# akanazawa/human_dynamics

Hardware: AMD Instinct MI355X
Metric: frames/sec/GPU (ResNet+temporal+SMPL, 224x224); SMPL verts max-abs-err (higher is better)
Workload: dtype f16x3

## Files before the change

### human_dynamics_amd/build.py

```python
from __future__ import annotations

import os
import subprocess
import sys
from concurrent.futures import ThreadPoolExecutor

HERE = os.path.dirname(os.path.abspath(__file__))
CSRC = os.path.join(HERE, "csrc")
INCLUDE = os.path.join(os.path.dirname(HERE), "include")
LIB = os.path.join(HERE, "libhmmr_hip.so")
SOURCES = ["api.cpp", "pack.cpp", "gemm_conv.hip", "conv3x3_stream.hip", "conv1x1_stream.hip", "stem.hip", "bottleneck.hip", "bottleneck_split.hip", "unit_pair.hip", "b1_unit.hip", "resnet.hip", "temporal.hip", "ief.hip", "ief_grad.hip", "movie_grad.hip", "smpl.hip", "smpl_grad.hip", "losses.hip", "eval_metrics.hip", "preprocess.hip", "tube.hip", "track.hip", "handoff.hip", "render.hip", "collage.hip", "person_view.hip", "windows.hip", "video_plan.cpp", "video.cpp", "probe.hip"]
HIPCC = os.environ.get("HIPCC", "/opt/rocm/bin/hipcc")
FLAGS = ["--offload-arch=gfx950", "-O3", "-std=c++17", "-fPIC", "-fno-slp-vectorize", "-I", INCLUDE, "-I", CSRC,
         "-Wall", "-Wno-unused-function"]


EXTRA_FLAGS = {"pack.cpp": ["-ffp-contract=off"], "track.hip": ["-ffp-contract=off"], "collage.hip": ["-ffp-contract=off"],
               "tube.hip": ["-ffp-contract=off"], "person_view.hip": ["-ffp-contract=off"]}


def _newer(src, dst):
    return (not os.path.exists(dst)) or os.path.getmtime(src) > os.path.getmtime(dst)


def _deps():
    return sorted(os.path.join(d, h) for d in (CSRC, INCLUDE) for h in os.listdir(d) if h.endswith(".h"))


def build(force=False, verbose=True):
    objs, jobs = [], []
    for src in SOURCES:
        s = os.path.join(CSRC, src)
        o = os.path.join(CSRC, os.path.splitext(src)[0] + ".o")
        objs.append(o)
# ... 34 lines not shown
```

### human_dynamics_amd/csrc/conv_tiles.h

```cpp
#pragma once
#include <stdio.h>

#include "hmmr_hip.h"


#define HMMR_GENERIC_TILES(X)                                                                                                         \
    X(1, 128, 128, 2, 2, 2, 0, 128, 0, 1, "128x128, 4 waves of 64x64")                                                                \
    X(2, 128, 64, 2, 2, 2, 0, 0, 0, 2, "128x64, 4 waves of 64x32")                                                                    \
    X(3, 64, 64, 2, 2, 2, 0, 0, 3, 3, "64x64, 4 waves of 32x32")                                                                      \
    X(5, 128, 128, 4, 2, 2, 0, 128, 1, 5, "128x128, 8 waves of 32x64, two workgroups per CU")                                         \
    X(6, 128, 64, 4, 2, 2, 0, 0, 2, 6, "128x64, 8 waves of 32x32, two workgroups per CU")                                             \
     \
     \
    X(7, 256, 128, 4, 2, 3, 0, 128, 0, 7, "256x128, 8 waves of 64x64, 3-stage ring, ping-pong wave groups")                           \
    X(8, 128, 256, 2, 4, 3, 256, 256, 0, 8, "128x256, likewise: half the A rows, half the fused-preact work per MFMA; the faster 3x3 tile")

#define HMMR_PATCH_TILES(X)                                                                                                           \
    X(9, 256, 128, 4, 2, 0, 128, 128, 1, 7, "256x128, the structure of tile 7 with the A operand out of an input patch")              \
    X(10, 128, 256, 2, 4, 0, 256, 256, 0, 8, "128x256, the structure of tile 8 likewise")                                             \
    X(11, 256, 128, 4, 2, 1, 128, 128, 0, 0, "256x128 without a load segment: two fragment sets per wave, one barrier per K step")

#define HMMR_S3_TILES(X)                                                                                                              \
    X(12, 7, 2, 2, 2, 28, 0, 128, 0, 1, 8, "448 pixels, waves 2 x 2")                                                                 \
    X(13, 4, 2, 2, 2, 28, 0, 128, 0, 2, 5, "256 pixels, waves 2 x 2")                                                                 \
    X(14, 8, 2, 2, 2, 28, 0, 128, 0, 0, 6, "512 pixels, waves 2 x 2")                                                                 \
    X(15, 6, 2, 2, 2, 28, 0, 128, 0, 3, 3, "384 pixels, waves 2 x 2")                                                                 \
    X(16, 5, 2, 2, 2, 28, 0, 128, 0, 4, 1, "320 pixels, waves 2 x 2")                                                                 \
    X(17, 4, 4, 4, 1, 28, 0, 128, 0, 0, 2, "512 pixels, the waves split the pixels")                                                  \
    X(18, 3, 4, 4, 1, 28, 0, 128, 0, 0, 7, "384 pixels, the waves split the pixels")                                                  \
    X(19, 5, 2, 4, 1, 56, 0, 64, 0, 8, 5, "640 pixels x 64 channels")                                                                 \
    X(20, 4, 2, 4, 1, 56, 0, 64, 0, 9, 6, "512 pixels x 64 channels")                                                                 \
    X(21, 7, 1, 1, 4, 28, 1, 128, 0, 5, 11, "224 pixels, every wave all of them and 32 of the 128 channels")                          \
     \
     \
    X(27, 2, 2, 2, 2, 28, 1, 128, 0, 6, 4, "128 pixels, waves 2 x 2: short launches")                                                 \
    X(28, 3, 2, 2, 2, 28, 1, 128, 0, 7, 9, "192 pixels, waves 2 x 2: short launches")

#define HMMR_S1_TILES(X)                                                                                                              \
    X(22, 7, 1, 1, 4, 6, 1, 0, 128, 0, 4, 5, "224 pixels, every wave all of them and 32 of the 128 channels")                         \
    X(23, 8, 1, 1, 4, 6, 1, 0, 128, 0, 5, 6, "256 pixels, likewise")                                                                  \
    X(24, 7, 2, 2, 2, 4, 1, 1, 128, 0, 2, 3, "448 pixels, waves 2 x 2")                                                               \
    X(25, 4, 2, 2, 2, 6, 1, 1, 128, 0, 1, 1, "256 pixels, waves 2 x 2")                                                               \
    X(26, 4, 2, 2, 2, 3, 2, 1, 128, 0, 3, 2, "256 pixels, waves 2 x 2, TWO workgroups per CU (rings 3 deep, 256 registers per wave)") \
     \
    X(29, 2, 2, 2, 2, 6, 1, 0, 128, 0, 6, 4, "128 pixels, waves 2 x 2: short launches")

#define HMMR_TILE_F_MOVIE 8

namespace conv_tiles {

constexpr hmmr_conv_tile_info_t make_row(int id, int family, int fm, int fn, int wgm, int wgn, int depth, int occ, int wmax, int split_only,
                                         int conv3_form, int cols, int tune, int rank, int cand, const char* text) {
    return {id, family, fm, fn, wgm, wgn, 32 * wgm * fm, 32 * wgn * fn, wgm * fm, depth, occ, wmax, split_only, conv3_form, cols, tune, cols == 64, rank, cand, text};
}

constexpr hmmr_conv_tile_info_t kRows[] = {
#define X(ID, BM, BN, WGM, WGN, NSTAGE, COLS, TUNE, RANK, CAND, TEXT) \
    make_row(ID, HMMR_TILE_GENERIC, BM / (32 * WGM), BN / (32 * WGN), WGM, WGN, NSTAGE, NSTAGE >= 3 ? 1 : 2, 0, 0, 0, COLS, TUNE, RANK, CAND, TEXT),
    HMMR_GENERIC_TILES(X)
#undef X
#define X(ID, BM, BN, WGM, WGN, PIPE, COLS, TUNE, RANK, CAND, TEXT) \
    make_row(ID, HMMR_TILE_PATCH, BM / (32 * WGM), BN / (32 * WGN), WGM, WGN, 3, 1, 0, PIPE, 0, COLS, TUNE, RANK, CAND, TEXT),
    HMMR_PATCH_TILES(X)
#undef X
#define X(ID, FM, FN, WGM, WGN, WMAX, SPLIT_ONLY, COLS, TUNE, RANK, CAND, TEXT) \
    make_row(ID, HMMR_TILE_STREAM_3X3, FM, FN, WGM, WGN, 0, 1, WMAX, SPLIT_ONLY, 0, COLS, TUNE, RANK, CAND, TEXT),
    HMMR_S3_TILES(X)
#undef X
#define X(ID, FM, FN, WGM, WGN, D, OCC, C3, COLS, TUNE, RANK, CAND, TEXT) \
    make_row(ID, HMMR_TILE_STREAM_1X1, FM, FN, WGM, WGN, D, OCC, 0, 0, C3, COLS, TUNE, RANK, CAND, TEXT),
    HMMR_S1_TILES(X)
#undef X
};
constexpr int kCount = (int)(sizeof(kRows) / sizeof(kRows[0]));

constexpr bool well_formed() {
    for (int i = 0; i < kCount; ++i) {
        const auto& a = kRows[i];
        if (a.tile < 1 || a.tile > HMMR_CONV_TILE_MAX || a.rank < 0 || a.candidate < 0) return false;
        int ranked_rows = 0;
        for (int j = 0; j < kCount; ++j) {
            const auto& b = kRows[j];
            if (b.family == a.family && b.rank > 0) ++ranked_rows;
            if (i == j) continue;
            if (a.tile == b.tile) return false;
            if (a.family != b.family) continue;
            if (a.rank && a.rank == b.rank) return false;
            if (a.candidate && a.candidate == b.candidate && a.narrow == b.narrow) return false;
        }
        if (a.rank > ranked_rows) return false;
    }
    return true;
}
static_assert(well_formed(), "conv_tiles.h: a tile number, a rank or a tuner candidate is used twice, or a number is out of range");

inline const hmmr_conv_tile_info_t* row(int tile) {
    for (const auto& r : kRows)
        if (r.tile == tile) return &r;
    return nullptr;
}

struct Ranked { int idx[kCount]; int n; };
constexpr Ranked ranked(int family) {
    Ranked o = {};
    for (int rank = 1; rank <= kCount; ++rank)
        for (int i = 0; i < kCount; ++i)
            if (kRows[i].family == family && kRows[i].rank == rank) o.idx[o.n++] = i;
    return o;
}

inline const char* list(int family, int narrow, char* buf, size_t n) {
    size_t at = 0;
    buf[0] = 0;
    for (int t = 1, end = 0; t <= HMMR_CONV_TILE_MAX; t = end + 1) {
        const auto in = [&](int id) { const auto* r = row(id); return r && r->family == family && (narrow < 0 || r->narrow == narrow); };
        end = t;
        if (!in(t)) continue;
        while (in(end + 1)) ++end;
        const int w = snprintf(buf + at, n - at, end >= t + 2 ? "%s%d .. %d" : end > t ? "%s%d, %d" : "%s%d", at ? ", " : "", t, end);
        if (w < 0 || (size_t)w >= n - at) break;
        at += (size_t)w;
    }
    return buf;
}
// ... 8 lines not shown
    int ksteps;
};
inline int family_of(int k_order, int filter_1x1) {
    return k_order == 2 ? (filter_1x1 ? HMMR_TILE_STREAM_1X1 : HMMR_TILE_STREAM_3X3) : k_order ? HMMR_TILE_PATCH : HMMR_TILE_GENERIC;
}
inline const char* family_name(int family) {
    static const char* const name[] = {"k_order 0", "k_order 1", "k_order 2", "k_order 2 (1x1)"};
    return name[family];
}

inline int fit(int tile, const Problem& p, char* why, size_t n) {
    const int fam = family_of(p.k_order, p.filter_1x1);
    const hmmr_conv_tile_info_t* t = row(tile);
    char ids[96];
    if (!t || t->family != fam) {
        snprintf(why, n, "%s runs tiles %s, not %d", family_name(fam), list(fam, -1, ids, sizeof ids), tile);
        return -1;
    }
    if (p.cout != 0 && (t->cols == 64 ? p.cout != 64 : t->cols && p.cout % t->cols)) {
        snprintf(why, n, "%s, tile %d (%s) needs cout %s %d, not %d (filter rows are padded to 128)", family_name(fam), tile, t->text,
                 t->cols == 64 ? "=" : "a multiple of", t->cols, p.cout);
        return -1;
    }
    if (t->split_only && p.dtype >= 0 && p.dtype != HMMR_F16X3) {
        snprintf(why, n, "%s, tile %d (%s) is built for split (f16x3) operands", family_name(fam), tile, t->text);
        return -1;
    }
    if (t->wmax && p.win > t->wmax) {
        snprintf(why, n, "%s, tile %d takes images up to %d pixels wide, not %d", family_name(fam), tile, t->wmax, p.win);
        return -1;
    }
    if (p.conv3_form && fam == HMMR_TILE_STREAM_1X1 && !t->conv3_form) {
        snprintf(why, n, "%s: tile %d (%s) has no conv3 form (res / out2 / in2)", family_name(fam), tile, t->text);
        return -1;
    }
    if (fam == HMMR_TILE_STREAM_1X1 && p.ksteps > 0 && p.ksteps < t->depth) {
        snprintf(why, n, "%s: cin must be at least %d channels for tile %d (rings %d K steps deep)", family_name(fam), 16 * t->depth, tile, t->depth);
        return -1;
    }
    return 0;
}

inline int tile_for(int k_order, int filter_1x1, int conv3_form, int cout, int dtype, int candidate) {
    const int fam = family_of(k_order, filter_1x1);
    const int narrow = fam == HMMR_TILE_STREAM_3X3 && cout == 64;
    const hmmr_conv_tile_info_t* t = nullptr;
    for (const auto& r : kRows)
        if (candidate > 0 && r.family == fam && r.narrow == narrow && r.candidate == candidate) { t = &r; break; }
    if (!t) t = row(candidate);
    if (!t || t->family != fam || t->narrow != narrow) return 0;
    if (t->split_only && dtype == HMMR_BF16) return 0;
    if (conv3_form && fam == HMMR_TILE_STREAM_1X1 && !t->conv3_form) return 0;
    if (t->tune_cols && cout % t->tune_cols) return 0;
    return t->tile;
}


inline int choose_generic(long long M, int cout, int slices) {
    constexpr Ranked rk = ranked(HMMR_TILE_GENERIC);
    for (int i = 0; i + 1 < rk.n; ++i) {
        const auto& r = kRows[rk.idx[i]];
        const long long tiles = ((M + r.pixels - 1) / r.pixels) * ((cout + r.channels - 1) / r.channels);
        const bool whole = r.channels < 128 || (cout >= r.channels && cout % r.channels == 0);
        if (whole && tiles * slices >= 192) return r.tile;
    }
    return kRows[rk.idx[rk.n - 1]].tile;
}

inline int choose_patch() { return kRows[ranked(HMMR_TILE_PATCH).idx[0]].tile; }

inline int choose_s3(long long M, int cout, bool split) {
    constexpr Ranked rk = ranked(HMMR_TILE_STREAM_3X3);
    const int narrow = cout == 64;
    const long long rbs = (M + 31) / 32, nts = narrow ? 1 : cout / 128;
    int tile = 0;
    double best = 0;
    for (int i = 0; i < rk.n; ++i) {
        const auto& r = kRows[rk.idx[i]];
        if (r.narrow != narrow || (r.split_only && !split)) continue;
        const long long tiles = ((rbs + r.row_blocks - 1) / r.row_blocks) * nts;
        const double cost = (double)((tiles + 255) / 256) * (r.row_blocks + 1.5);
        if (!tile || cost < best) { tile = r.tile; best = cost; }
    }
    return tile;
}

inline int choose_s1(long long M, int cout, int nk, bool c3) {
    constexpr Ranked rk = ranked(HMMR_TILE_STREAM_1X1);
    const long long rbs = (M + 31) / 32, tiles_n = cout / 128;
    int tile = 0;
    double best = 0;
    for (int i = 0; i < rk.n; ++i) {
        const auto& r = kRows[rk.idx[i]];
        if (nk < r.depth || (c3 && !r.conv3_form)) continue;
        const long long tiles = ((rbs + r.row_blocks - 1) / r.row_blocks) * tiles_n;
        double cost = (double)((tiles + 255) / 256) * (r.row_blocks + 1.5) * (r.tile == 22 || r.tile == 23 ? 1.15 : 1.0);
        if (r.tile == 26) cost = (double)((tiles + 511) / 512) * 2.0 * (r.row_blocks + 1.5) * (c3 ? 0.8 : nk <= 32 ? 0.88 : 1.05);
        if (!tile || cost < best) { tile = r.tile; best = cost; }
    }
    return tile;
}

constexpr int s1_min_depth() {
    int d = 1 << 30;
    for (const auto& r : kRows)
        if (r.family == HMMR_TILE_STREAM_1X1 && r.depth < d) d = r.depth;
    return d;
}

// ... 2 lines not shown
```

### human_dynamics_amd/csrc/gemm_conv.hip

```cpp
#include <stdlib.h>
#include <string.h>
#include <type_traits>

#include "conv_tiles.h"
#include "stream_kit.h"

struct ConvArgs {
    const void* in; const void* w; const float* scale; const float* shift;
    const void* res; void* out; void* out2; const float* scale2; const float* shift2;
    const float* pro_scale; const float* pro_shift;
    void* out_b; int ldo_b, n_split, relu_b;
    int M, K, cout, ldo, ldr;
    int Wo, HoWo, Hin, Win;
    long long in_img_stride; int in_row_stride, in_px_stride;
    int cin_log2, KH, KW, SY, SX, PY, PX;
    int res_strided; long long res_img_stride; int res_row_stride, res_px_stride;
    int relu, tiles_n, n_tiles;
    int kt_per_slice;
    long long out_slice_stride;
    int probe;
    const void* in2; int cin2, kt_split;
    int batch; long long bz_in, bz_w, bz_out, bz_res, bz_scale, bz_shift;
};

// ... 875 lines not shown
#undef X
        default: hmmr_set_error("hmmr_conv_gemm: k_order 1: no tile %d", tile); return -1;
    }
}

template <typename TA, typename TO, int BM, int BN, int WGM, int WGN, bool PRO, bool UTAP, int NSTAGE>
static int launch_cfg(const ConvArgs& base, int slices, hipStream_t stream) {
    ConvArgs a = base;
    const int tiles_m = (a.M + BM - 1) / BM;
    a.tiles_n = (a.cout + BN - 1) / BN;
    a.n_tiles = tiles_m * a.tiles_n;
    constexpr int kring = NSTAGE * (BM + BN) * 128, epi = BM * BN * 4;
    const int kloop = kring + ((PRO && NSTAGE >= 3) ? 8 * a.K : 0);
    const int lds = kloop > epi ? kloop : epi;
    if (lds > 160 * 1024) { hmmr_set_error("hmmr_conv_gemm: tile needs %d B of LDS (K = %d)", lds, a.K); return -1; }
    auto kern = conv_gemm_kernel<TA, TO, BM, BN, WGM, WGN, PRO, UTAP, NSTAGE>;
    static DeviceOnce once;
    constexpr int BKE_ = 8 * elem_traits<TA>::EPS;
    const int nk = a.K / BKE_;
    a.kt_per_slice = (nk + slices - 1) / slices;
    return launch_with_lds(kern, once, dim3(a.n_tiles, slices, a.batch), dim3(WGM * WGN * 64), NSTAGE >= 3 ? 160 * 1024 : lds, lds, stream, a);
}

template <typename TA, typename TO, bool PRO, bool UTAP>
static int launch_tiled(const ConvArgs& a, int tile, int slices, hipStream_t stream) {
    switch (tile) {
#define X(ID, BM, BN, WGM, WGN, NSTAGE, ...) case ID: return launch_cfg<TA, TO, BM, BN, WGM, WGN, PRO, UTAP, NSTAGE>(a, slices, stream);
        HMMR_GENERIC_TILES(X)
#undef X
        default: hmmr_set_error("hmmr_conv_gemm: k_order 0: no tile %d", tile); return -1;
    }
}

template <typename TA, typename TO>
static int launch_typed(const ConvArgs& a, int tile, int slices, hipStream_t stream) {
    if (tile == 0) tile = conv_tiles::choose_generic(a.M, a.cout, slices);
    char why[256];
    HMMR_REQUIRE(!conv_tiles::fit(tile, conv_tiles::Problem{0, 0, 0, a.cout, -1, 0, 0}, why, sizeof why), "hmmr_conv_gemm: %s", why);
    const bool utap = ((size_t)1 << a.cin_log2) * sizeof(TA) >= 128;
    if (a.pro_scale) {
        if (!utap) { hmmr_set_error("hmmr_conv_gemm: fused pre-activation needs cin*sizeof >= 128"); return -1; }
        return launch_tiled<TA, TO, true, true>(a, tile, slices, stream);
    }
    return utap ? launch_tiled<TA, TO, false, true>(a, tile, slices, stream)
                : launch_tiled<TA, TO, false, false>(a, tile, slices, stream);
}

template <typename TO>
__global__ __launch_bounds__(256) void splitk_reduce_kernel(const ConvArgs a0, const float* __restrict__ part,
                                                            int slices, int ldw, long long plane) {
// ... 57 lines not shown
#pragma unroll
        for (int j = 0; j < 8; ++j) {
            const float vr = stored_value<TO>(v[j]);
            u[j] = fmaxf(fmaf(vr, s2[j], b2[j]), 0.f);
        }
        if (full) store8(out2 + oo, u);
        else store_tail(out2 + oo, u, a.cout - n);
    }
}

extern "C" size_t hmmr_conv_splitk_workspace_bytes(int m, int cout, int split_k) {
    if (split_k <= 1 || m <= 0) return 0;
    return (size_t)split_k * (size_t)m * (size_t)((cout + 127) / 128 * 128) * sizeof(float);
}

static int ilog2_exact(int v) {
    int l = 0;
    while ((1 << l) < v) ++l;
    return ((1 << l) == v) ? l : -1;
}

int hmmr_conv3x3_stream(const hmmr_conv_desc_t* d, hipStream_t stream);
int hmmr_conv1x1_stream(const hmmr_conv_desc_t* d, hipStream_t stream);

extern "C" int hmmr_conv_gemm(const hmmr_conv_desc_t* d, void* stream) {
    HMMR_REQUIRE(d && d->in && d->w && (d->out || d->out2), "hmmr_conv_gemm: null operand");
    const int esz = d->in_dtype == HMMR_BF16 ? 2 : 4;
    const int eps = d->in_dtype == HMMR_F16X3 ? 8 : 16 / esz;
    const int cl2 = ilog2_exact(d->cin);
    HMMR_REQUIRE(cl2 >= 0 && d->cin % eps == 0, "hmmr_conv_gemm: cin=%d must be a power of two >= %d", d->cin, eps);
    const int K = d->kh * d->kw * d->cin + (d->in2 ? d->cin2 : 0);
    HMMR_REQUIRE(d->kh * d->kw <= 32, "hmmr_conv_gemm: at most 32 filter taps");
    const int bke = 128 / esz;
    HMMR_REQUIRE(K % bke == 0, "hmmr_conv_gemm: K=%d must be a multiple of %d", K, bke);
    HMMR_REQUIRE(d->out_dtype != HMMR_F16X3 || d->cout % 8 == 0,
                 "hmmr_conv_gemm: a split (f16x3) output needs cout %% 8 == 0 (rows are whole hi/lo groups)");
    HMMR_REQUIRE(d->ldo % 8 == 0, "hmmr_conv_gemm: ldo=%d must be a multiple of 8", d->ldo);
    const bool px_ok = d->in_px_stride % eps == 0 ||
                       (d->kw == 1 && d->px == 0 && (d->in_px_stride * d->sx) % eps == 0);
    HMMR_REQUIRE(px_ok && d->in_row_stride % eps == 0 && d->in_img_stride % eps == 0,
                 "hmmr_conv_gemm: input strides must keep 16-byte alignment");
    HMMR_REQUIRE(!d->res || d->res_strided || d->ldr % 8 == 0, "hmmr_conv_gemm: ldr must be a multiple of 8");
    HMMR_REQUIRE(!d->res || d->cout % 8 == 0 || (!d->res_strided && d->ldr >= (d->cout + 7) / 8 * 8),
                 "hmmr_conv_gemm: residual rows must be readable up to cout rounded up to 8");
    HMMR_REQUIRE(!d->out2 || (d->scale2 && d->shift2), "hmmr_conv_gemm: out2 needs scale2/shift2");
    HMMR_REQUIRE(!d->pro_scale == !d->pro_shift, "hmmr_conv_gemm: pro_scale and pro_shift go together");
// ... 18 lines not shown
    a.pro_scale = d->pro_scale; a.pro_shift = d->pro_shift;
    a.out_b = d->out_b; a.ldo_b = d->ldo_b; a.n_split = d->n_split; a.relu_b = d->relu_b;
    a.M = d->n_img * d->ho * d->wo; a.K = K; a.cout = d->cout; a.ldo = d->ldo; a.ldr = d->ldr;
    a.Wo = d->wo; a.HoWo = d->ho * d->wo; a.Hin = d->hin; a.Win = d->win;
    a.in_img_stride = d->in_img_stride; a.in_row_stride = d->in_row_stride; a.in_px_stride = d->in_px_stride;
    a.cin_log2 = cl2; a.KH = d->kh; a.KW = d->kw; a.SY = d->sy; a.SX = d->sx; a.PY = d->py; a.PX = d->px;
    a.res_strided = d->res_strided; a.res_img_stride = d->res_img_stride;
    a.res_row_stride = d->res_row_stride; a.res_px_stride = d->res_px_stride;
    a.relu = d->relu; a.tiles_n = 0; a.n_tiles = 0;
    a.kt_per_slice = 0; a.out_slice_stride = 0; a.probe = 0;
    a.in2 = d->in2; a.cin2 = d->in2 ? d->cin2 : 0; a.kt_split = d->cin / bke;
    a.batch = d->batch > 1 ? d->batch : 1;
    a.bz_in = d->batch_in_bytes; a.bz_w = d->batch_w_bytes; a.bz_out = d->batch_out_bytes;
    a.bz_res = d->batch_res_bytes; a.bz_scale = d->batch_scale_bytes; a.bz_shift = d->batch_shift_bytes;
    HMMR_REQUIRE(a.batch == 1 || (a.batch <= 64 && !d->k_order && !d->out_b && !d->in2 && !d->pro_scale &&
                                  ((d->batch_in_bytes | d->batch_w_bytes | d->batch_out_bytes | d->batch_res_bytes | d->batch_scale_bytes | d->batch_shift_bytes) & 15) == 0),
                 "hmmr_conv_gemm: a grouped launch (batch > 1) takes up to 64 problems, strides that are multiples of 16 bytes, "
                 "and no k_order / out_b / in2 / pro_scale");
#ifdef HMMR_GEMM_PROBE
    a.probe = hmmr_debug_state()->gemm_probe;
#endif
    if (a.M <= 0) return 0;
    hipStream_t s = (hipStream_t)stream;
    if (d->k_order == 2 && d->kh == 1 && d->kw == 1) return hmmr_conv1x1_stream(d, s);
    if (d->k_order) {
        HMMR_REQUIRE((d->k_order == 1 || d->k_order == 2) && d->kh == 3 && d->kw == 3 && d->sy == 1 && d->sx == 1 && d->py == 1 && d->px == 1 &&
                     d->ho == d->hin && d->wo == d->win && d->in_px_stride == d->cin && d->in_row_stride == d->win * d->cin &&
                     d->in_img_stride == (int64_t)d->hin * d->win * d->cin && (d->cin * esz) % 128 == 0 &&
                     !d->res && !d->out2 && !d->out_b && !d->pro_scale && !d->in2 && d->split_k <= 1 && d->out && d->cout % 8 == 0,
                     "hmmr_conv_gemm: k_order 1 is for 3x3 / stride 1 / pad 1 convolutions over a dense NHWC tensor with "
                     "cin a multiple of the 128-byte K step and a scale/shift/relu epilogue (no res, out2, out_b, pro_scale, in2, split_k)");
        if (d->k_order == 2) return hmmr_conv3x3_stream(d, s);
        const bool px3 = d->in_dtype == HMMR_F16X3 && d->out_dtype == HMMR_F16X3, pbf = d->in_dtype == HMMR_BF16 && d->out_dtype == HMMR_BF16;
        HMMR_REQUIRE(px3 || pbf, "hmmr_conv_gemm: k_order 1 is built for split (f16x3) and bf16 tensors");
        const int ptile = d->tile ? d->tile : conv_tiles::choose_patch();
        HMMR_REQUIRE(!conv_tiles::fit(ptile, conv_tiles::Problem{1, 0, 0, d->cout, d->in_dtype, 0, 0}, why, sizeof why), "hmmr_conv_gemm: %s", why);
        if (pbf) return launch_patch_tiled<bf16_t, bf16_t>(a, ptile, s);
        return launch_patch_tiled<bsplit_t, bsplit_t>(a, ptile, s);
    }
    const bool in16 = d->in_dtype == HMMR_BF16, in32 = d->in_dtype == HMMR_F32, inx3 = d->in_dtype == HMMR_F16X3;
    const bool out16 = d->out_dtype == HMMR_BF16, out32 = d->out_dtype == HMMR_F32, outx3 = d->out_dtype == HMMR_F16X3;
    HMMR_REQUIRE((in16 || in32 || inx3) && (out16 || out32 || outx3), "hmmr_conv_gemm: unsupported dtypes %d -> %d", d->in_dtype, d->out_dtype);
    const int nk = K / bke;
    int slices = d->split_k > 1 ? d->split_k : 1;
    if (slices > nk) slices = nk;
    slices = (nk + ((nk + slices - 1) / slices) - 1) / ((nk + slices - 1) / slices);
// ... 33 lines not shown
```

### human_dynamics_amd/csrc/resnet.hip

```cpp
#include <stdlib.h>

#include <type_traits>

#include "common.h"
#include "hmmr_hip.h"
#include "workspace.h"

int hmmr_stem_fused(const float* images, int n_real, int n, const void* wts, const float* wscale, const float* bias,
                    const float* pscale, const float* pshift, void* out, int dtype, hipStream_t s,
                    const void* w1, const float* s1, const float* b1, void* out_h1);

static constexpr int IMG = 224, PADH = 230, PADW = 232;

__global__ void stem_repack_split_kernel(const float* __restrict__ img, bsplit_t* __restrict__ out, long long npairs,
                                         long long n_real) {
    for (long long i = (long long)blockIdx.x * blockDim.x + threadIdx.x; i < npairs;
         i += (long long)gridDim.x * blockDim.x) {
        const int xp = (int)(i % (PADW / 2));
        const long long t = i / (PADW / 2);
        const int y = (int)(t % PADH);
        const long long n = t / PADH;
        float v[8];
#pragma unroll
        for (int e = 0; e < 8; ++e) v[e] = 0.f;
        const int sy = y - 3;
        if (n < n_real && (unsigned)sy < (unsigned)IMG) {
#pragma unroll
// ... 329 lines not shown
        const T* res = p.shortcut == HMMR_SC_NONE ? X[cur] : xn;
        const int res_stride = p.shortcut == HMMR_SC_NONE ? U.stride : 1;
        hmmr_conv_desc_t d;
        if (p.shortcut == HMMR_SC_LAUNCH || p.shortcut == HMMR_SC_LAUNCH_WITH_CONV1) {
            d = dense_conv(dt, n, xin, H, U.c_in, 1, U.stride, U.depth, U.shortcut, xn);
            d.pro_scale = ps; d.pro_shift = pb;
            d.k_order = 0;
            if (p.shortcut == HMMR_SC_LAUNCH_WITH_CONV1) {
                d.w = U.sc_c1.w; d.scale = U.sc_c1.scale; d.shift = U.sc_c1.shift; d.k_order = U.sc_c1.k_order;
                d.cout = U.depth + U.base; d.out_b = T1; d.ldo_b = U.base; d.n_split = U.depth; d.relu_b = 1;
            }
            if (hmmr_conv_gemm(&d, s)) return -2;
        }
        if (p.shortcut != HMMR_SC_NONE && prof_mark(pf)) return -2;
        if (p.conv1 == HMMR_CONV1_LAUNCH) {
            d = dense_conv(dt, n, xin, H, U.c_in, 1, 1, U.base, U.conv1, T1);
            d.pro_scale = ps; d.pro_shift = pb; d.relu = 1;
            if (hmmr_conv_gemm(&d, s)) return -2;
        }
        if (prof_mark(pf)) return -2;
        if (p.conv2 == HMMR_CONV2_LAUNCH) {
            d = dense_conv(dt, n, T1, H, U.base, 3, U.stride, U.base, U.conv2, T2);
            d.relu = 1;
            if (hmmr_conv_gemm(&d, s)) return -2;
        }
        if (prof_mark(pf)) return -2;
        if (p.end == HMMR_END_CONV3_LAUNCH) {
            d = dense_conv(dt, n, T2, Ho, U.base, 1, 1, U.depth, sc_in_c3 ? U.c3sc : U.conv3, out);
            if (sc_in_c3) { d.in2 = xin; d.cin2 = U.c_in; } else set_residual(d, res, U.depth, H, res_stride);
            if (pre) { d.out2 = pre; d.scale2 = N.pre_scale; d.shift2 = N.pre_shift; }
            if (hmmr_conv_gemm(&d, s)) return -2;
        } else {
            hmmr_tail_desc_t t = {};
            t.dtype = dt; t.m = n * Ho * Ho; t.c_mid = U.base; t.depth = U.depth; t.ho = t.wo = Ho;
            t.w3 = U.conv3.w; t.scale3 = U.conv3.scale; t.shift3 = U.conv3.shift;
            if (p.conv2 == HMMR_CONV2_IN_TAIL) {
                t.h1 = T1; t.hin = t.win = H; t.w2 = U.conv2.w; t.scale2 = U.conv2.scale; t.shift2 = U.conv2.shift;
            } else t.h2 = T2;
            if (p.end == HMMR_END_TAIL_BF16_STRIDE2) {
                t.conv2_stride = U.stride;
                set_residual(t, res, U.depth, H, res_stride);
                t.out = out; t.out_pre = pre;
                if (pre) { t.pre_scale = N.pre_scale; t.pre_shift = N.pre_shift; }
            } else {
                if (dt == HMMR_F16X3) {
                    t.w3 = U.w3_frag;
// ... 71 lines not shown
```

Before: 39310.

## Add dedicated streaming kernel for stride-2 3x3 convolutions on split tensors

Adds a new kernel for 3x3 stride-2 pad-1 convolutions on f16x3 tensors. It streams filter and input pixel slabs into LDS rings several stages deep with direct global-to-LDS loads, zero-pads the top and left edges from a zero page, and interleaves fragment reads with MFMAs. Adds tile rows and a chooser for it. Dispatch sends matching convolutions with no tile set to it by default, in place of the generic implicit GEMM path. This adds a large hand-scheduled kernel with tight vmcnt and LDS budget assumptions.

```diff
diff --git a/human_dynamics_amd/build.py b/human_dynamics_amd/build.py
--- a/human_dynamics_amd/build.py
+++ b/human_dynamics_amd/build.py
@@ -9,7 +9,7 @@
 CSRC = os.path.join(HERE, "csrc")
 INCLUDE = os.path.join(os.path.dirname(HERE), "include")
 LIB = os.path.join(HERE, "libhmmr_hip.so")
-SOURCES = ["api.cpp", "pack.cpp", "gemm_conv.hip", "conv3x3_stream.hip", "conv1x1_stream.hip", "stem.hip", "bottleneck.hip", "bottleneck_split.hip", "unit_pair.hip", "b1_unit.hip", "resnet.hip", "temporal.hip", "ief.hip", "ief_grad.hip", "movie_grad.hip", "smpl.hip", "smpl_grad.hip", "losses.hip", "eval_metrics.hip", "preprocess.hip", "tube.hip", "track.hip", "handoff.hip", "render.hip", "collage.hip", "person_view.hip", "windows.hip", "video_plan.cpp", "video.cpp", "probe.hip"]
+SOURCES = ["api.cpp", "pack.cpp", "gemm_conv.hip", "conv3x3_stream.hip", "conv1x1_stream.hip", "conv3x3_s2_stream.hip", "stem.hip", "bottleneck.hip", "bottleneck_split.hip", "unit_pair.hip", "b1_unit.hip", "resnet.hip", "temporal.hip", "ief.hip", "ief_grad.hip", "movie_grad.hip", "smpl.hip", "smpl_grad.hip", "losses.hip", "eval_metrics.hip", "preprocess.hip", "tube.hip", "track.hip", "handoff.hip", "render.hip", "collage.hip", "person_view.hip", "windows.hip", "video_plan.cpp", "video.cpp", "probe.hip"]
 HIPCC = os.environ.get("HIPCC", "/opt/rocm/bin/hipcc")
 FLAGS = ["--offload-arch=gfx950", "-O3", "-std=c++17", "-fPIC", "-fno-slp-vectorize", "-I", INCLUDE, "-I", CSRC,
          "-Wall", "-Wno-unused-function"]
diff --git a/human_dynamics_amd/csrc/conv3x3_s2_stream.hip b/human_dynamics_amd/csrc/conv3x3_s2_stream.hip
--- /dev/null
+++ b/human_dynamics_amd/csrc/conv3x3_s2_stream.hip
@@ -0,0 +1,324 @@
+#include "conv_tiles.h"
+#include "stream_kit.h"
+
+namespace {
+
+__device__ const u32x4 g_s2_zero_page[4] = {};
+
+struct S2Args {
+    const char* in;
+    const char* w;
+    const float* scale; const float* shift;
+    void* out; int ldo, relu;
+    int M, W, C, Wo, HoWo;
+    int nc_log2, nk;
+    int tiles_n, n_tiles;
+};
+
+__device__ __forceinline__ unsigned long long uniform64(unsigned long long v) {
+    const unsigned lo = (unsigned)__builtin_amdgcn_readfirstlane((int)(unsigned)v), hi = (unsigned)__builtin_amdgcn_readfirstlane((int)(unsigned)(v >> 32));
+    return ((unsigned long long)hi << 32) | lo;
+}
+
+template <typename F, int... S> __device__ __forceinline__ void s2_group(F&& f, int kt0, int nk, std::integer_sequence<int, S...>) {
+    ((kt0 + S < nk ? f(ic<S>{}, kt0 + S) : (void)0), ...);
+}
+
+template <int FM, int FN, int WGM, int WGN, int D>
+__global__ __launch_bounds__(256, conv_tiles::s2_occupancy(32 * WGM * FM, 32 * WGN * FN, D)) void conv3x3_s2_stream_kernel(const S2Args a) {
+    constexpr int NB = WGN * FN;
+    static_assert(WGM * WGN == 4 && (NB == 4 || NB == 2) && FM * FN <= 16 && D >= 3 && D <= 6, "4 waves, 128 or 64 channels, at most 16 accumulators");
+    constexpr int U = D % 2 ? 2 * D : D;
+    constexpr int R = WGM * FM, BM = 32 * R;
+    static_assert(BM % 64 == 0, "pixel slabs are whole 64-row pieces");
+    constexpr int NPX = BM / 64;
+    constexpr int XSLAB = BM * 64;
+    constexpr int SLAB = NB * 2048, RING = D * SLAB;
+    constexpr int RW = NB / 2;
+    constexpr int P = RW + NPX;
+    constexpr int CST = RING + D * XSLAB;
+    constexpr int NR = 2 * (FM + FN), NG = 3 * FM * FN;
+    static_assert(CST + 2048 == conv_tiles::s2_lds_bytes(BM, 32 * NB, D) && CST + 2048 <= 160 * 1024 && 4 * 8192 <= CST, "LDS; the epilogue's staging tiles live in the idle rings");
+    static_assert(D * P < 64, "vmcnt");
+    static_assert(2048 * (FM - 1) + 16 < 65536 && (D - 1) * SLAB + (FN - 1) * 2048 + 16 < 65536, "instruction offsets");
+    static_assert(NR <= NG && NPX + 1 <= NG, "a gap for every fragment read and every pixel request");
+
+    extern __shared__ __attribute__((aligned(256))) char smem[];
+    const int tid = threadIdx.x, lane = tid & 63;
+    const int wave = __builtin_amdgcn_readfirstlane(tid >> 6);
+    const int lr = lane & 31, lh = lane >> 5;
+    const int L = xcd_remap(blockIdx.x, a.n_tiles);
+    const int mt = L / a.tiles_n, nt = L - mt * a.tiles_n;
+    const int m0 = mt * BM;
+    const int nk = a.nk;
+    const int wm = wave / WGN, wn = wave - wm * WGN;
+    const unsigned lds0 = lds_addr(smem);
+
+    float cv = 0.f;
+    if (tid < 64 * NB) cv = tid < 32 * NB ? a.scale[nt * (32 * NB) + tid] : a.shift[nt * (32 * NB) + tid - 32 * NB];
+
+    const int img0 = m0 / a.HoWo;
+    const int Hin2 = 2 * (a.HoWo / a.Wo);
+    int poff[NPX];
+    unsigned pout[NPX];
+#pragma unroll
+    for (int q = 0; q < NPX; ++q) {
+        const int r = 64 * q + 16 * wave + (lane >> 2);
+        int m = m0 + r;
+        m = m >= a.M ? a.M - 1 : m;
+        const int img = m / a.HoWo, rem = m - img * a.HoWo;
+        const int oy = rem / a.Wo, ox = rem - oy * a.Wo;
+        poff[q] = (((img - img0) * Hin2 + 2 * oy - 1) * a.W + 2 * ox - 1) * (a.C * 4) + (((lane & 3) ^ ((r >> 2) & 3)) << 4);
+        pout[q] = (oy == 0 ? 1u : 0u) | (ox == 0 ? 2u : 0u);
+    }
+    const unsigned long long in_t = (unsigned long long)a.in + (unsigned long long)img0 * (unsigned long long)Hin2 * (unsigned long long)(a.W * a.C * 4);
+    const char* const zero = (const char*)g_s2_zero_page;
+    auto x_base = [&](int s, unsigned& sel) {
+        const int tap = s >> a.nc_log2, c = s - (tap << a.nc_log2);
+        const int ky = (tap * 11) >> 5, kx = tap - 3 * ky;
+        sel = (ky == 0 ? 1u : 0u) | (kx == 0 ? 2u : 0u);
+        return (const char*)uniform64(in_t + (unsigned long long)(long long)((ky * a.W + kx) * (a.C * 4) + c * 64));
+    };
+    auto x_piece = [&](int q, const char* xb, unsigned sel, int slot) {
+        char* dst = smem + RING + slot * XSLAB + q * 4096 + wave * 1024;
+        const char* src = (pout[q] & sel) ? zero : xb + (long long)poff[q];
+        __builtin_amdgcn_global_load_lds((gptr_t)src, (lptr_t)dst, 16, 0, 0);
+    };
+    const unsigned kbytes = 9u * (unsigned)a.C * 4u;
+    unsigned woff[RW];
+#pragma unroll
+    for (int p = 0; p < RW; ++p) {
+        const unsigned r = 64u * p + 16u * wave + ((unsigned)lane >> 2);
+        woff[p] = r * kbytes + ((((unsigned)lane & 3u) ^ ((r >> 2) & 3u)) << 4);
+    }
+    const unsigned long long w_t = (unsigned long long)a.w + (unsigned long long)(nt * (32 * NB)) * (unsigned long long)kbytes;
+    auto ring_dma = [&](int s, int slot) {
+        const unsigned long long wb = uniform64(w_t + (unsigned long long)(s * 64));
+        char* dst = smem + slot * SLAB + wave * 1024;
+#pragma unroll
+        for (int p = 0; p < RW; ++p) __builtin_amdgcn_global_load_lds((gptr_t)((const char*)wb + woff[p]), (lptr_t)(dst + p * 4096), 16, 0, 0);
+    };
+    __builtin_amdgcn_sched_barrier(0);
+#pragma unroll
+    for (int s_ = 0; s_ < D; ++s_) {
+        const int sp = s_ < nk ? s_ : nk - 1;
+        ring_dma(sp, s_);
+        unsigned sel;
+        const char* xb = x_base(sp, sel);
+#pragma unroll
+        for (int q = 0; q < NPX; ++q) x_piece(q, xb, sel, s_);
+    }
+    __builtin_amdgcn_sched_barrier(0);
+    if (tid < 64 * NB) ((float*)(smem + CST))[tid] = cv;
+
+    f32x16 acc[FM][FN];
+#pragma unroll
+    for (int i = 0; i < FM; ++i)
+#pragma unroll
+        for (int j = 0; j < FN; ++j) {
+#pragma unroll
+            for (int r = 0; r < 16; ++r) acc[i][j][r] = 0.f;
+            asm volatile("" : "+a"(acc[i][j]));
+        }
+
+    const unsigned wr0 = (unsigned)(wn * FN * 32 + lr);
+    const unsigned aw = lds0 + wr0 * 64 + (((2u * lh) ^ ((wr0 >> 2) & 3u)) << 4), awl = aw ^ 16u;
+    const unsigned rb0 = (unsigned)(wm * FM * 32 + lr);
+    const unsigned ax0 = lds0 + RING + rb0 * 64 + (((2u * lh) ^ ((rb0 >> 2) & 3u)) << 4);
+    xfrag fx[2][FM];
+    wfrag fw[2][FN];
+    unsigned adcur = 0, adcurl = 0;
+
+    auto read_one = [&](int set, int r, int slot_) {
+        if (r < 2 * FN) {
+            const int j = r >> 1, pl = r & 1;
+#define S2_F(SL, J, PL) if (slot_ == SL && j == J && pl == PL) { shalf8 v = lds_rd128<shalf8, SL * SLAB + J * 2048>(PL ? awl : aw); if (PL) fw[set][J].lo = v; else fw[set][J].hi = v; }
+#define S2_FJ(SL, J) S2_F(SL, J, 0) S2_F(SL, J, 1)
+#define S2_FS(SL) if constexpr (SL < D) { S2_FJ(SL, 0) if constexpr (FN > 1) { S2_FJ(SL, 1) } }
+            S2_FS(0) S2_FS(1) S2_FS(2) S2_FS(3) S2_FS(4) S2_FS(5)
+#undef S2_FS
+#undef S2_FJ
+#undef S2_F
+        } else {
+            const int i = (r - 2 * FN) >> 1, pl = (r - 2 * FN) & 1;
+#define S2_X(I) if constexpr (I < FM) { if (i == I) { if (pl) fx[set][I].lo = lds_rd128<shalf8, I * 2048>(adcurl); else fx[set][I].hi = lds_rd128<shalf8, I * 2048>(adcur); } }
+            S2_X(0) S2_X(1) S2_X(2) S2_X(3) S2_X(4) S2_X(5) S2_X(6) S2_X(7)
+#undef S2_X
+        }
+    };
+    static_assert(FN <= 2 && FM <= 8, "read_one spells out two filter and eight pixel fragments");
+    auto slot_setup = [&](int slot_) {
+        adcur = ax0 + slot_ * XSLAB;
+        adcurl = adcur ^ 16u;
+    };
+    constexpr auto gap_of = [](int r) { return NR <= NG - 4 ? 2 + (r * (NG - 4)) / NR : r / 2; };
+
+    __builtin_amdgcn_sched_barrier(0);
+    wait_vm_lgkm0<(D - 1) * P>();
+    __builtin_amdgcn_s_barrier();
+    __builtin_amdgcn_sched_barrier(0);
+    slot_setup(0);
+#pragma unroll
+    for (int r = 0; r < NR; ++r) read_one(0, r, 0);
+    __builtin_amdgcn_sched_barrier(0);
+    wait_vm_lgkm0<(D - 2) * P>();
+    __builtin_amdgcn_s_barrier();
+    __builtin_amdgcn_sched_barrier(0);
+
+    auto step = [&](auto s_c, int kt) {
+        constexpr int S = decltype(s_c)::value, CUR = S & 1, NXT = CUR ^ 1, SNEXT = (S + 1) % D;
+        const int sn = kt + D < nk ? kt + D : nk - 1;
+        unsigned sel;
+        const char* xsrc = x_base(sn, sel);
+#pragma unroll
+        for (int i = 0; i < FM; ++i)
+#pragma unroll
+            for (int p = 0; p < 3; ++p)
+#pragma unroll
+                for (int j = 0; j < FN; ++j) {
+                    const shalf8& wa = p == 1 ? fw[CUR][j].lo : fw[CUR][j].hi;
+                    const shalf8& xb = p == 0 ? fx[CUR][i].lo : fx[CUR][i].hi;
+                    acc[i][j] = mfma_split(wa, xb, acc[i][j]);
+                    const int g = (3 * i + p) * FN + j;
+                    if (g == 0) { ring_dma(sn, S % D); slot_setup(SNEXT); }
+                    if (g >= 1 && g < 1 + NPX) x_piece(g - 1 < NPX ? g - 1 : 0, xsrc, sel, S % D);
+#pragma unroll
+                    for (int r = 0; r < NR; ++r)
+                        if (gap_of(r) == g) read_one(NXT, r, SNEXT);
+                    __builtin_amdgcn_sched_barrier(0);
+                }
+        wait_vm_lgkm0<(D - 2) * P>();
+        __builtin_amdgcn_sched_barrier(0);
+        __builtin_amdgcn_s_barrier();
+        __builtin_amdgcn_sched_barrier(0);
+    };
+    for (int kt0 = 0; kt0 < nk; kt0 += U) s2_group(step, kt0, nk, std::make_integer_sequence<int, U>{});
+    __builtin_amdgcn_sched_barrier(0);
+    wait_vm_lgkm0<0>();
+    __builtin_amdgcn_s_barrier();
+    __builtin_amdgcn_sched_barrier(0);
+
+    char* stg = smem + wave * 8192;
+    const int rsub = lane >> 3, pslot = lane & 7, sw = (lr >> 1) & 7;
+    const int nb = nt * (32 * NB) + wn * FN * 32;
+    f32x4 s4[FN][4], b4[FN][4];
+    {
+        const float* cst = (const float*)(smem + CST) + wn * FN * 32 + 4 * lh;
+#pragma unroll
+        for (int j = 0; j < FN; ++j)
+#pragma unroll
+            for (int g = 0; g < 4; ++g) {
+                s4[j][g] = *(const f32x4*)(cst + j * 32 + 8 * g);
+                b4[j][g] = *(const f32x4*)(cst + 32 * NB + j * 32 + 8 * g);
+            }
+    }
+    float satmax = 0.f;
+    int blk = 0;
+#pragma unroll
+    for (int i = 0; i < FM; ++i) {
+        const int mb = m0 + (wm * FM + i) * 32;
+        bsplit_t* orow[4];
+#pragma unroll
+        for (int q = 0; q < 4; ++q) {
+            const int r = 8 * q + rsub, m = mb + r;
+            const int ls = pslot ^ ((r >> 1) & 7);
+            orow[q] = m < a.M ? (bsplit_t*)a.out + (long long)m * a.ldo + nb + ls * 4 : (bsplit_t*)g_dump_page + lane * 4;
+        }
+#pragma unroll
+        for (int j = 0; j < FN; ++j, ++blk) {
+            char* tile = stg + (blk & 1) * 4096;
+#pragma unroll
+            for (int g = 0; g < 4; ++g) {
+                float c[4];
+#pragma unroll
+                for (int e = 0; e < 4; ++e) {
+                    float v = fmaf(acc[i][j][4 * g + e], s4[j][g][e], b4[j][g][e]);
+                    if (a.relu) v = fmaxf(v, 0.f);
+                    satmax = sat_acc(satmax, v);
+                    c[e] = split_clamp(v);
+                }
+                unsigned h01, l01, h23, l23;
+                split2_mix(c[0], c[1], h01, l01);
+                split2_mix(c[2], c[3], h23, l23);
+                const unsigned long long oh = (unsigned long long)h01 | ((unsigned long long)h23 << 32);
+                const unsigned long long ol = (unsigned long long)l01 | ((unsigned long long)l23 << 32);
+                stage_store_group(tile, lr, lh, g, sw, oh, ol);
+            }
+            u32x4 xr[4];
+#pragma unroll
+            for (int q = 0; q < 4; ++q) xr[q] = *(const u32x4*)(tile + q * 1024 + lane * 16);
+#pragma unroll
+            for (int q = 0; q < 4; ++q) *(u32x4*)(orow[q] + j * 32) = xr[q];
+        }
+    }
+    split_flag_max(satmax);
+}
+
+template <int FM, int FN, int WGM, int WGN, int D>
+int launch_s2(const S2Args& base, hipStream_t stream) {
+    S2Args a = base;
+    constexpr int NB = WGN * FN, BM = 32 * WGM * FM;
+    constexpr int lds = conv_tiles::s2_lds_bytes(BM, 32 * NB, D);
+    a.tiles_n = a.tiles_n / NB;
+    a.n_tiles = ((a.M + BM - 1) / BM) * a.tiles_n;
+    auto kern = conv3x3_s2_stream_kernel<FM, FN, WGM, WGN, D>;
+    static DeviceOnce once;
+    return launch_with_lds(kern, once, dim3((unsigned)a.n_tiles), dim3(256), lds, lds, stream, a);
+}
+
+template <int BM, int BN, int WGM, int WGN, int D>
+int launch_s2_row(const S2Args& a, int tile, hipStream_t stream) {
+    if constexpr (conv_tiles::s2_shape(WGM * WGN, D)) return launch_s2<BM / (32 * WGM), BN / (32 * WGN), WGM, WGN, D>(a, stream);
+    else { hmmr_set_error("hmmr_conv_gemm: tile %d is no tile of the stride-2 3x3 stream kernel", tile); return -1; }
+}
+
+constexpr int s2_max_pixels() {
+    int m = 0;
+    for (const auto& r : conv_tiles::kRows)
+        if (conv_tiles::is_s2(r) && r.pixels > m) m = r.pixels;
+    return m;
+}
+
+}
+
+const char* hmmr_conv3x3_s2_misses(const hmmr_conv_desc_t* d) {
+    if (d->k_order || d->kh != 3 || d->kw != 3 || d->sy != 2 || d->sx != 2 || d->py != 1 || d->px != 1)
+        return "a 3x3 / stride 2 / pad 1 convolution with k_order 0";
+    if (d->hin < 2 || d->win < 2 || d->hin % 2 || d->win % 2 || d->ho != d->hin / 2 || d->wo != d->win / 2)
+        return "an image of even height and width (only the top row and the left column of taps may leave it), ho = hin / 2, wo = win / 2";
+    if (d->in_dtype != HMMR_F16X3 || d->out_dtype != HMMR_F16X3) return "split (f16x3) tensors in and out";
+    if (d->cin < 16 || d->cin % 16 || !(d->cout == 64 || (d->cout > 0 && d->cout % 128 == 0))) return "cin a multiple of 16 and cout = 64 or a multiple of 128";
+    if (d->in_px_stride != d->cin || d->in_row_stride != d->win * d->cin || d->in_img_stride != (int64_t)d->hin * d->win * d->cin)
+        return "a dense NHWC input tensor";
+    if (!d->scale || !d->shift || !d->out) return "scale, shift and out";
+    if (d->res || d->out2 || d->in2 || d->pro_scale || d->out_b || d->split_k > 1 || d->batch > 1)
+        return "no res, out2, in2, pro_scale, out_b, split_k or batch";
+    const long long M = (long long)d->n_img * d->ho * d->wo, howo = (long long)d->ho * d->wo;
+    const long long span = ((long long)s2_max_pixels() / howo + 3) * d->hin * d->win * d->cin * 4;
+    if (M >= (1ll << 31) || span >= (1ll << 31) || (long long)d->cout * 9 * d->cin * 4 >= (1ll << 31)) return "fewer than 2^31 pixels, and images and a filter bank below 2 GB";
+    return nullptr;
+}
+
+int hmmr_conv3x3_s2_stream(const hmmr_conv_desc_t* d, hipStream_t stream) {
+    const char* miss = hmmr_conv3x3_s2_misses(d);
+    HMMR_REQUIRE(!miss, "hmmr_conv_gemm: tile %d (the stride-2 3x3 stream kernel) needs %s", d->tile, miss);
+    const long long M = (long long)d->n_img * d->ho * d->wo;
+    if (M <= 0) return 0;
+    const int tile = d->tile ? d->tile : conv_tiles::choose_s2(M, d->cout);
+    char why[256];
+    HMMR_REQUIRE(!conv_tiles::fit(tile, conv_tiles::Problem{0, 0, 0, d->cout, d->in_dtype, 0, 0}, why, sizeof why), "hmmr_conv_gemm: %s", why);
+    S2Args a = {};
+    a.in = (const char*)d->in; a.w = (const char*)d->w; a.scale = d->scale; a.shift = d->shift;
+    a.out = d->out; a.ldo = d->ldo; a.relu = d->relu;
+    a.M = (int)M; a.W = d->win; a.C = d->cin; a.Wo = d->wo; a.HoWo = d->ho * d->wo;
+    int l2 = 0;
+    while ((16 << l2) < d->cin) ++l2;
+    a.nc_log2 = l2; a.nk = 9 << l2;
+    a.tiles_n = d->cout / 32;
+    switch (tile) {
+#define X(ID, BM, BN, WGM, WGN, NSTAGE, ...) case ID: return launch_s2_row<BM, BN, WGM, WGN, NSTAGE>(a, tile, stream);
+        HMMR_GENERIC_TILES(X)
+#undef X
+        default: hmmr_set_error("hmmr_conv_gemm: k_order 0: no tile %d", tile); return -1;
+    }
+}
diff --git a/human_dynamics_amd/csrc/conv_tiles.h b/human_dynamics_amd/csrc/conv_tiles.h
--- a/human_dynamics_amd/csrc/conv_tiles.h
+++ b/human_dynamics_amd/csrc/conv_tiles.h
@@ -13,7 +13,12 @@
      \
      \
     X(7, 256, 128, 4, 2, 3, 0, 128, 0, 7, "256x128, 8 waves of 64x64, 3-stage ring, ping-pong wave groups")                           \
-    X(8, 128, 256, 2, 4, 3, 256, 256, 0, 8, "128x256, likewise: half the A rows, half the fused-preact work per MFMA; the faster 3x3 tile")
+    X(8, 128, 256, 2, 4, 3, 256, 256, 0, 8, "128x256, likewise: half the A rows, half the fused-preact work per MFMA; the faster 3x3 tile")    \
+    X(31, 256, 128, 2, 2, 6, 128, 128, 4, 4, "stride-2 3x3 stream: 256 pixels x 128, waves 2 x 2, rings 6 deep")                       \
+    X(32, 128, 128, 2, 2, 4, 128, 128, 5, 11, "stride-2 3x3 stream: 128 pixels x 128, rings 4 deep")                                  \
+    X(33, 64, 128, 2, 2, 6, 128, 128, 6, 0, "stride-2 3x3 stream: 64 pixels x 128, waves 2 x 2: short launches")                        \
+    X(34, 512, 64, 4, 1, 4, 64, 64, 7, 4, "stride-2 3x3 stream: 512 pixels x 64, every wave both 32-column blocks, rings 4 deep")       \
+    X(35, 256, 64, 4, 1, 3, 64, 64, 8, 11, "stride-2 3x3 stream: 256 pixels x 64, likewise, rings 3 deep")
 
 #define HMMR_PATCH_TILES(X)                                                                                                           \
     X(9, 256, 128, 4, 2, 0, 128, 128, 1, 7, "256x128, the structure of tile 7 with the A operand out of an input patch")              \
@@ -49,6 +54,10 @@
 
 namespace conv_tiles {
 
+constexpr bool s2_shape(int waves, int stages) { return waves == 4 && stages >= 3; }
+constexpr int s2_lds_bytes(int bm, int bn, int stages) { return stages * (bm + bn) * 64 + 2048; }
+constexpr int s2_occupancy(int bm, int bn, int stages) { return 2 * s2_lds_bytes(bm, bn, stages) <= 160 * 1024 ? 2 : 1; }
+
 constexpr hmmr_conv_tile_info_t make_row(int id, int family, int fm, int fn, int wgm, int wgn, int depth, int occ, int wmax, int split_only,
                                          int conv3_form, int cols, int tune, int rank, int cand, const char* text) {
     return {id, family, fm, fn, wgm, wgn, 32 * wgm * fm, 32 * wgn * fn, wgm * fm, depth, occ, wmax, split_only, conv3_form, cols, tune, cols == 64, rank, cand, text};
@@ -56,7 +65,7 @@
 
 constexpr hmmr_conv_tile_info_t kRows[] = {
 #define X(ID, BM, BN, WGM, WGN, NSTAGE, COLS, TUNE, RANK, CAND, TEXT) \
-    make_row(ID, HMMR_TILE_GENERIC, BM / (32 * WGM), BN / (32 * WGN), WGM, WGN, NSTAGE, NSTAGE >= 3 ? 1 : 2, 0, 0, 0, COLS, TUNE, RANK, CAND, TEXT),
+    make_row(ID, HMMR_TILE_GENERIC, BM / (32 * WGM), BN / (32 * WGN), WGM, WGN, NSTAGE, s2_shape(WGM * WGN, NSTAGE) ? s2_occupancy(BM, BN, NSTAGE) : NSTAGE >= 3 ? 1 : 2, 0, s2_shape(WGM * WGN, NSTAGE), 0, COLS, TUNE, RANK, CAND, TEXT),
     HMMR_GENERIC_TILES(X)
 #undef X
 #define X(ID, BM, BN, WGM, WGN, PIPE, COLS, TUNE, RANK, CAND, TEXT) \
@@ -100,6 +109,8 @@
     return nullptr;
 }
 
+constexpr bool is_s2(const hmmr_conv_tile_info_t& r) { return r.family == HMMR_TILE_GENERIC && r.split_only; }
+
 struct Ranked { int idx[kCount]; int n; };
 constexpr Ranked ranked(int family) {
     Ranked o = {};
@@ -154,6 +165,10 @@
                  t->cols == 64 ? "=" : "a multiple of", t->cols, p.cout);
         return -1;
     }
+    if (is_s2(*t) && (p.filter_1x1 || p.conv3_form)) {
+        snprintf(why, n, "%s, tile %d (%s) takes 3x3 / stride 2 / pad 1 convolutions only", family_name(fam), tile, t->text);
+        return -1;
+    }
     if (t->split_only && p.dtype >= 0 && p.dtype != HMMR_F16X3) {
         snprintf(why, n, "%s, tile %d (%s) is built for split (f16x3) operands", family_name(fam), tile, t->text);
         return -1;
@@ -176,11 +191,16 @@
 inline int tile_for(int k_order, int filter_1x1, int conv3_form, int cout, int dtype, int candidate) {
     const int fam = family_of(k_order, filter_1x1);
     const int narrow = fam == HMMR_TILE_STREAM_3X3 && cout == 64;
+    const bool s2_class = fam == HMMR_TILE_GENERIC && !filter_1x1 && !conv3_form && dtype == HMMR_F16X3 && (cout == 64 || (cout > 0 && cout % 128 == 0));
     const hmmr_conv_tile_info_t* t = nullptr;
-    for (const auto& r : kRows)
-        if (candidate > 0 && r.family == fam && r.narrow == narrow && r.candidate == candidate) { t = &r; break; }
+    for (const auto& r : kRows) {
+        if (candidate <= 0 || r.family != fam || r.candidate != candidate) continue;
+        if (is_s2(r) ? (s2_class && r.narrow == (cout == 64)) : r.narrow == narrow) { t = &r; break; }
+    }
     if (!t) t = row(candidate);
-    if (!t || t->family != fam || t->narrow != narrow) return 0;
+    if (!t || t->family != fam) return 0;
+    if (is_s2(*t)) return s2_class && t->narrow == (cout == 64) ? t->tile : 0;
+    if (t->narrow != narrow) return 0;
     if (t->split_only && dtype == HMMR_BF16) return 0;
     if (conv3_form && fam == HMMR_TILE_STREAM_1X1 && !t->conv3_form) return 0;
     if (t->tune_cols && cout % t->tune_cols) return 0;
@@ -188,8 +208,14 @@
 }
 
 
+constexpr Ranked ranked_gemm() {
+    Ranked all = ranked(HMMR_TILE_GENERIC), o = {};
+    for (int i = 0; i < all.n; ++i)
+        if (!is_s2(kRows[all.idx[i]])) o.idx[o.n++] = all.idx[i];
+    return o;
+}
 inline int choose_generic(long long M, int cout, int slices) {
-    constexpr Ranked rk = ranked(HMMR_TILE_GENERIC);
+    constexpr Ranked rk = ranked_gemm();
     for (int i = 0; i + 1 < rk.n; ++i) {
         const auto& r = kRows[rk.idx[i]];
         const long long tiles = ((M + r.pixels - 1) / r.pixels) * ((cout + r.channels - 1) / r.channels);
@@ -217,6 +243,22 @@
     return tile;
 }
 
+inline int choose_s2(long long M, int cout) {
+    constexpr Ranked rk = ranked(HMMR_TILE_GENERIC);
+    const int narrow = cout == 64;
+    const long long rbs = (M + 31) / 32, nts = narrow ? 1 : cout / 128;
+    int tile = 0;
+    double best = 0;
+    for (int i = 0; i < rk.n; ++i) {
+        const auto& r = kRows[rk.idx[i]];
+        if (!is_s2(r) || r.narrow != narrow) continue;
+        const long long tiles = ((rbs + r.row_blocks - 1) / r.row_blocks) * nts;
+        const double cost = (double)((tiles + 255) / 256) * (r.row_blocks + 1.5) * (r.occupancy == 2 && tiles > 256 ? 0.9 : 1.0);
+        if (!tile || cost < best) { tile = r.tile; best = cost; }
+    }
+    return tile;
+}
+
 inline int choose_s1(long long M, int cout, int nk, bool c3) {
     constexpr Ranked rk = ranked(HMMR_TILE_STREAM_1X1);
     const long long rbs = (M + 31) / 32, tiles_n = cout / 128;
diff --git a/human_dynamics_amd/csrc/gemm_conv.hip b/human_dynamics_amd/csrc/gemm_conv.hip
--- a/human_dynamics_amd/csrc/gemm_conv.hip
+++ b/human_dynamics_amd/csrc/gemm_conv.hip
@@ -921,10 +921,16 @@
     return launch_with_lds(kern, once, dim3(a.n_tiles, slices, a.batch), dim3(WGM * WGN * 64), NSTAGE >= 3 ? 160 * 1024 : lds, lds, stream, a);
 }
 
+template <typename TA, typename TO, int BM, int BN, int WGM, int WGN, bool PRO, bool UTAP, int NSTAGE>
+static int launch_row(const ConvArgs& a, int tile, int slices, hipStream_t stream) {
+    if constexpr (conv_tiles::s2_shape(WGM * WGN, NSTAGE)) { hmmr_set_error("hmmr_conv_gemm: k_order 0: tile %d is the stride-2 3x3 stream kernel's", tile); return -1; }
+    else return launch_cfg<TA, TO, BM, BN, WGM, WGN, PRO, UTAP, NSTAGE>(a, slices, stream);
+}
+
 template <typename TA, typename TO, bool PRO, bool UTAP>
 static int launch_tiled(const ConvArgs& a, int tile, int slices, hipStream_t stream) {
     switch (tile) {
-#define X(ID, BM, BN, WGM, WGN, NSTAGE, ...) case ID: return launch_cfg<TA, TO, BM, BN, WGM, WGN, PRO, UTAP, NSTAGE>(a, slices, stream);
+#define X(ID, BM, BN, WGM, WGN, NSTAGE, ...) case ID: return launch_row<TA, TO, BM, BN, WGM, WGN, PRO, UTAP, NSTAGE>(a, tile, slices, stream);
         HMMR_GENERIC_TILES(X)
 #undef X
         default: hmmr_set_error("hmmr_conv_gemm: k_order 0: no tile %d", tile); return -1;
@@ -1028,6 +1034,8 @@
 
 int hmmr_conv3x3_stream(const hmmr_conv_desc_t* d, hipStream_t stream);
 int hmmr_conv1x1_stream(const hmmr_conv_desc_t* d, hipStream_t stream);
+int hmmr_conv3x3_s2_stream(const hmmr_conv_desc_t* d, hipStream_t stream);
+const char* hmmr_conv3x3_s2_misses(const hmmr_conv_desc_t* d);
 
 extern "C" int hmmr_conv_gemm(const hmmr_conv_desc_t* d, void* stream) {
     HMMR_REQUIRE(d && d->in && d->w && (d->out || d->out2), "hmmr_conv_gemm: null operand");
@@ -1092,6 +1100,8 @@
 #endif
     if (a.M <= 0) return 0;
     hipStream_t s = (hipStream_t)stream;
+    if (const hmmr_conv_tile_info_t* t = conv_tiles::row(d->tile); !d->k_order && (t ? conv_tiles::is_s2(*t) : !d->tile && !hmmr_conv3x3_s2_misses(d)))
+        return hmmr_conv3x3_s2_stream(d, s);
     if (d->k_order == 2 && d->kh == 1 && d->kw == 1) return hmmr_conv1x1_stream(d, s);
     if (d->k_order) {
         HMMR_REQUIRE((d->k_order == 1 || d->k_order == 2) && d->kh == 3 && d->kw == 3 && d->sy == 1 && d->sx == 1 && d->py == 1 && d->px == 1 &&
diff --git a/human_dynamics_amd/csrc/resnet.hip b/human_dynamics_amd/csrc/resnet.hip
--- a/human_dynamics_amd/csrc/resnet.hip
+++ b/human_dynamics_amd/csrc/resnet.hip
@@ -3,6 +3,7 @@
 #include <type_traits>
 
 #include "common.h"
+#include "conv_tiles.h"
 #include "hmmr_hip.h"
 #include "workspace.h"
 
@@ -378,6 +379,7 @@
         if (p.conv2 == HMMR_CONV2_LAUNCH) {
             d = dense_conv(dt, n, T1, H, U.base, 3, U.stride, U.base, U.conv2, T2);
             d.relu = 1;
+            if (const hmmr_conv_tile_info_t* t = conv_tiles::row(d.tile); U.stride == 1 && t && conv_tiles::is_s2(*t)) d.tile = 0;
             if (hmmr_conv_gemm(&d, s)) return -2;
         }
         if (prof_mark(pf)) return -2;
```

Result: no change. 39490, median of 6 (+0.4%).
